# conanhujinming/flash_hash_join

Hardware: AMD Instinct MI355X
Metric: probe throughput (billion probes/sec), int64 keys, whole join (build + probe phases) per step (higher is better)
Workload: dtype int64

## Files before the change

flash_hash_join_amd/_lib.py:

```python
from __future__ import annotations

import ctypes
import os
import subprocess

_PKG = os.path.dirname(os.path.abspath(__file__))
VARIANT = os.environ.get("FJ_LIB_VARIANT", "")
LIB_PATH = (os.path.join(_PKG, "lib", "libflashjoin_hip.so") if not VARIANT
            else os.path.join(_PKG, "lib", "libflashjoin_hip_lab.so") if VARIANT == "lab"
            else os.path.join(_PKG, "lib", "ab", VARIANT + ".so"))
PRODUCT_LIB_PATH = os.path.join(_PKG, "lib", "libflashjoin_hip.so")
LAB_LIB_PATH = os.path.join(_PKG, "lib", "libflashjoin_hip_lab.so")
ABI_VERSION = 8
CSRC = os.path.join(_PKG, "csrc")

SYMBOLS = [
    "fj_initialize", "fj_last_error", "fj_device_count", "fj_version", "fj_abi_version", "fj_set_option", "fj_get_option", "fj_key_mix64", "fj_key_unmix64",
    "fj_ctx_create", "fj_ctx_destroy", "fj_ctx_workspace_bytes", "fj_ctx_trim",
    "fj_join_host", "fj_free_host", "fj_last_timings", "fj_join_device", "fj_emit_pairs",
    "fj_owner_split", "fj_stream_abort", "fj_shuffle_plan", "fj_bcast_plan",
    "fj_dist_comm_set_form", "fj_dist_model", "fj_dist_unique_id", "fj_dist_comm_create", "fj_dist_comm_from_nccl", "fj_dist_comm_from_transport",
    "fj_dist_comm_destroy", "fj_dist_comm_rank", "fj_dist_comm_size", "fj_dist_join_count", "fj_dist_join",
    "fj_generate_build", "fj_generate_probe",
    "fj_device_malloc", "fj_device_free", "fj_memcpy_h2d", "fj_memcpy_d2h", "fj_memcpy_d2d",
]
LAB_SYMBOLS = [
    "fj_owner_hist", "fj_owner_scatter",
    "fj_shuffle_chunk_bytes", "fj_shuffle_pack_begin", "fj_shuffle_pack_counts", "fj_shuffle_pack_finish", "fj_stream_open_shuffled",
    "fj_stream_append_build_chunks", "fj_stream_append_probe_chunks",
    "fj_shuffle_part_filter_bytes", "fj_shuffle_part_filter_range", "fj_stream_export_part_filters", "fj_shuffle_pack_filter", "fj_shuffle_pack_kept", "fj_part_filter_sample",
    "fj_bcast_region_bytes", "fj_bcast_piece_span", "fj_bcast_pack", "fj_bcast_pack_bounds", "fj_bcast_probe", "fj_bcast_join", "fj_bcast_finish", "fj_bcast_abort",
    "fj_bloom_filter_words", "fj_bloom_export", "fj_bloom_prefilter",
    "fj_stream_open", "fj_stream_append_build", "fj_stream_advance_probe", "fj_stream_begin", "fj_stream_append_probe", "fj_stream_finish",
    "fj_ctx_reserve_cus", "fj_key_pair64", "fj_debug_partition",
]


class FjTimings(ctypes.Structure):
    _fields_ = [
        ("total_ms", ctypes.c_double), ("build_phase_ms", ctypes.c_double), ("probe_phase_ms", ctypes.c_double),
        ("join_ms", ctypes.c_double), ("emit_ms", ctypes.c_double), ("probe_part_kernel_ms", ctypes.c_double * 4),
        ("h2d_ms", ctypes.c_double), ("d2h_ms", ctypes.c_double),
        ("path", ctypes.c_int), ("passes", ctypes.c_int), ("radix_bits", ctypes.c_int), ("fell_back", ctypes.c_int),
        ("partitions", ctypes.c_uint64), ("overlapped", ctypes.c_int), ("lds_retries", ctypes.c_int),
        ("filter_ms", ctypes.c_double), ("filter_survivors", ctypes.c_uint64), ("bloom_level", ctypes.c_int), ("sampled_hit_bp", ctypes.c_int), ("host_streamed", ctypes.c_int), ("reserved3", ctypes.c_int),
    ]

    def as_dict(self):
        d = {n: getattr(self, n) for n, _ in self._fields_ if n != "probe_part_kernel_ms"}
        d["probe_part_kernel_ms"] = list(self.probe_part_kernel_ms)
        return d


class FjDistTimings(ctypes.Structure):
    _fields_ = [
        ("struct_size", ctypes.c_size_t),
        ("total_ms", ctypes.c_double), ("split_ms", ctypes.c_double), ("exchange_ms", ctypes.c_double), ("join_ms", ctypes.c_double),
# ... 149 lines not shown
        L.fj_shuffle_chunk_bytes.restype = sz; L.fj_shuffle_chunk_bytes.argtypes = [sz, i32]
        L.fj_shuffle_pack_begin.restype = i32; L.fj_shuffle_pack_begin.argtypes = [vp, vp, vp, sz, sz, i32, i32, vp]
        L.fj_shuffle_part_filter_bytes.restype = sz; L.fj_shuffle_part_filter_bytes.argtypes = []
        L.fj_shuffle_part_filter_range.restype = i32; L.fj_shuffle_part_filter_range.argtypes = [sz, i32, i32, ctypes.POINTER(sz), ctypes.POINTER(sz), ctypes.POINTER(sz)]
        L.fj_stream_export_part_filters.restype = i32; L.fj_stream_export_part_filters.argtypes = [vp, vp, vp]
        L.fj_shuffle_pack_filter.restype = i32; L.fj_shuffle_pack_filter.argtypes = [vp, vp, vp]
        L.fj_shuffle_pack_kept.restype = u64; L.fj_shuffle_pack_kept.argtypes = [vp]
        L.fj_part_filter_sample.restype = i32; L.fj_part_filter_sample.argtypes = [vp, vp, sz, sz, vp, sz, i32, vp, pu64]
        L.fj_shuffle_pack_counts.restype = i32; L.fj_shuffle_pack_counts.argtypes = [vp, pu64]
        L.fj_shuffle_pack_finish.restype = i32; L.fj_shuffle_pack_finish.argtypes = [vp, ctypes.POINTER(vp), ctypes.POINTER(vp), ctypes.POINTER(vp), vp]
        L.fj_stream_open_shuffled.restype = i32; L.fj_stream_open_shuffled.argtypes = [vp, sz, i32, i32, sz, i32, sz, i32, i32, vp]
        L.fj_stream_append_build_chunks.restype = i32; L.fj_stream_append_build_chunks.argtypes = [vp, vp, vp, vp, sz, vp]
        L.fj_stream_append_probe_chunks.restype = i32; L.fj_stream_append_probe_chunks.argtypes = [vp, vp, vp, sz, vp]
        L.fj_bcast_region_bytes.restype = sz; L.fj_bcast_region_bytes.argtypes = [sz, sz, i32]
        L.fj_bcast_piece_span.restype = i32; L.fj_bcast_piece_span.argtypes = [sz, sz, sz, sz, i32, psz, psz]
        L.fj_bcast_pack.restype = i32; L.fj_bcast_pack.argtypes = [vp, vp, vp, sz, sz, vp, i32, i32, vp]
        L.fj_bcast_pack_bounds.restype = i32; L.fj_bcast_pack_bounds.argtypes = [vp, pu64]
        L.fj_bcast_probe.restype = i32; L.fj_bcast_probe.argtypes = [vp, vp, sz, sz, vp]
        L.fj_bcast_join.restype = i32; L.fj_bcast_join.argtypes = [vp, vp, i32, pu64, pu64, ctypes.c_uint32, ctypes.c_uint32, vp]
        L.fj_bcast_finish.restype = i32; L.fj_bcast_finish.argtypes = [vp, vp, pu64, ctypes.POINTER(FjTimings)]
        L.fj_bcast_abort.restype = None; L.fj_bcast_abort.argtypes = [vp]
        if hasattr(L, "fj_key_pair64"):
            L.fj_key_pair64.restype = u64; L.fj_key_pair64.argtypes = [u64, u64]
        L.fj_debug_partition.restype = i32
        L.fj_debug_partition.argtypes = [vp, vp, vp, sz, i32, i32, vp, vp, vp, vp, pu64]
    _lib = L
    return L


def last_error() -> str:
    return load().fj_last_error().decode("utf-8", "replace")


def check(rc: int) -> None:
    if rc != 0:
        msg = last_error()
        if "out of" in msg and "memory" in msg:
            raise MemoryError(msg)
        raise RuntimeError(msg)
```

flash_hash_join_amd/csrc/fj_host.h:

```cpp
#pragma once
#include "fj_internal.h"
#include "../../include/flashjoin.h"
#include "../../include/flashjoin_lab.h"

#include <algorithm>
#include <chrono>
#include <cstdarg>
#include <cstdio>
#include <cstdlib>
#include <cstring>
#include <condition_variable>
#include <functional>
#include <mutex>
#include <string>
#include <thread>
#include <vector>

struct StreamState;

namespace fjh {

int set_err(const char* fmt, ...);
fj_timings& last_timings();
#define HIPCHK(x)                                                                                          \
// ... 86 lines not shown

struct Prepared {
    enum Form { EMPTY, LDS, HBM };
    bool valid = false;
    Form form = EMPTY;
    bool has_vals = false;
    int top_bits = 64, path = 0;
    Plan plan; u32 nparts = 0;
    size_t nb = 0; u64 g = 0;
    u64* keys = nullptr; u64* rows = nullptr; u64* vals = nullptr; void* aux = nullptr;
    u64 cap_mask = 0;
    size_t bytes = 0;
};

struct PassIter {
    int side = 0; bool has_vals = false; size_t n = 0; Plan plan; int used = 64; u32 parents = 1; u64 lbound = 0;
    u32 tile_chunks = 16; int i = 0;
    FjChunkSet prev{}; bool have_prev = false; const uint4* tiles = nullptr; const u32* ntiles = nullptr; const u32* toff = nullptr;
    FjChunkSet cs{}; u32 Gmax = 1, F = 1, appends = 1;
    size_t piece_rows = 0;
    int slot = 0, cs_base = 0;
    u32 item_tc_max = 0;
    bool want_items = false; u32 items_cap = 0; u32* part_count = nullptr; int part_count_slot = W_PART_COUNT;
    bool bloom_done = false; const FjChunkSet* bloom_build = nullptr;
    const u32* bloom_prebuilt = nullptr;
    unsigned long long* bloom_bucket_keys = nullptr;
    int save_level = 0; FjChunkSet saved{};
    u32* alloc_word = nullptr; u32* seg_word = nullptr; u32* err_word = nullptr;
    bool in_pk7 = false; u32 in_b0 = 0, in_top_shift = 0;
    bool vals_pos = false;
};

}

struct PackState {
    bool begun = false, deferred = false;
    u32 part_shift = 0;
    fjh::PassIter it;
    FjPackArgs args{};
    int nranks = 0;
};

struct StreamState {
    bool active = false;
    fjh::Plan plan; fjh::PassIter pit, bit; FjLdsJoinArgs ja{};
    int top_bits = 64, evc = 0;
// ... 18 lines not shown
};

struct fj_ctx {
    int device = 0;
    fjh::Buf bufs[fjh::W_NSLOTS];
    hipEvent_t ev[fjh::E_NEV];
    hipStream_t side = nullptr;
    fjh::Scalars* d_sc = nullptr;
    fjh::Scalars* h_sc = nullptr;
    fjh::Pending pend;
    fjh::Prepared prep;
    StreamState st;
    PackState pk;
    BcastState bc;
    hipEvent_t pk_ev = nullptr;
    unsigned long long* pk_h = nullptr;
    size_t ws_bytes = 0;
    u32 num_cus = 256;
    u32 reserve_cus = 0;
    void* stage[3] = {nullptr, nullptr, nullptr};
    size_t stage_bytes = 0;
    bool plan_in_flight = false;
    bool slot_dirty[fjh::W_NSLOTS] = {};
    std::recursive_mutex mu;
};

namespace fjh {

#define FJ_HOOK_LOOPBACK 1
#define FJ_HOOK_INJECT_FAIL 2
#define FJ_HOOK_SPLIT_ALWAYS 4
#define FJ_HOOK_ONE_COMM 8
#define FJ_HOOK_RESERVE_ALWAYS 16
#define FJ_HOOK_EMIT_TAGGED 32
#define FJ_HOOK_EMIT_RETRY_7TH 64
struct Options {
    size_t radix_threshold = 0; int scalar_hbm_table = 0; u32 persistent_min_items = 8192; u32 plan_target_keys = FJ_PART_TARGET_KEYS;
    int bloom_variant = 0, bloom_auto = 1, bloom_auto_max_hit_bp = 2300, mat_single_pass = 1;
    int join_wide = 2;
    u32 lab_hooks = 0;
    u32 join_items_target = 2048;
    int mm_heavy_keys = 0;
    int mm_heavy_outer = 0;
    Options();
};
Options& options();

int get_buf(fj_ctx* c, int slot, size_t bytes, void** out);
int get_zeroed_buf(fj_ctx* c, int slot, size_t bytes, void** out, hipStream_t s);
int plan_npass(int bits);
void plan_passes(Plan& p, bool extra_first);
Plan make_plan(size_t nb, int top_bits, bool want_bloom = false, u64 target_override = 0);
void pass_init(PassIter& it, int side, bool has_vals, size_t n, const Plan& plan, int top_bits);
u32 pass_groups(u64 chunks, u64 rows, u32 tile_chunks, u32 F);
int pass_prepare(fj_ctx* c, PassIter& it, u32 appends, hipStream_t s);
int pass_launch(fj_ctx* c, PassIter& it, const u64* keys, const u64* vals, size_t n, hipStream_t s, int* ev_cursor);
bool bloom_stage_follows(const PassIter& it, int level);
void join_item_geometry(u64 nparts, size_t np, u64 chunk_bound, u32* tc, u64* max_items);
bool wide_join_planned(bool materialize, size_t nb, size_t np_eff, int bits);
int level_finish(fj_ctx* c, PassIter& it, bool final_level, hipStream_t s);
int pass_complete(fj_ctx* c, PassIter& it, hipStream_t s);
int bloom_stage(fj_ctx* c, PassIter& it, hipStream_t s);
int run_passes(fj_ctx* c, PassIter& it, const u64* keys, const u64* vals, hipStream_t s, FjChunkSet* out, int* ev_cursor);
int clear_plan_scalars(fj_ctx* c, hipStream_t s);
void begin_plan(fj_ctx* c);
void end_plan(fj_ctx* c);
void drop_pending(fj_ctx* c);
int begin_step(fj_ctx* c, const char* who);
int read_scalars(fj_ctx* c, hipStream_t s);
float ev_ms(fj_ctx* c, int a, int b);
void plan_timings(fj_ctx* c, const Plan& plan, u64 partitions, int evc, fj_timings* t);
int stamps_begin(unsigned long long** dbg, hipStream_t s);
int stamps_report(const char* label, const unsigned long long* dbg, u32 nitems, hipStream_t s);

int emit_pending(fj_ctx* c, u64* d_ok, u64* d_ov, size_t cap, hipStream_t s, fj_timings* t);
int radix_join_tail(fj_ctx* c, int materialize, FjLdsJoinArgs& ja, const Plan& plan, size_t np, const PassIter& pit, hipStream_t s,
                    fj_timings* t, int evc, u64* out_count, bool* lds_full, int top_bits, SingleOut* so = nullptr);

int join_outer(fj_ctx* c, int mode, bool use_radix, const u64* bk, const u64* bv, size_t nb, const u64* pk, size_t np, int top_bits,
               hipStream_t s, fj_timings* t, u64* out_count, u64* d_ok, u64* d_ov, bool rid = false);
int join_full(fj_ctx* c, bool use_radix, const u64* bk, const u64* bv, size_t nb, const u64* pk, size_t np, int top_bits,
// ... 42 lines not shown
```

flash_hash_join_amd/csrc/fj_internal.h:

```cpp
#pragma once
#include "fj_common.h"

#define FJ_ERR_POOL 1u
#define FJ_ERR_LDS_FULL 2u
#define FJ_STAT_DUPS 4u
#define FJ_STAT_RETRY 8u
#define FJ_STAT_EMIT_RETRY 16u
#define FJ_ERR_VARIANT 32u
#define FJ_BLOOM_HDR_MAGIC 0xB100F000u
#define FJ_STAT_TOOBIG 64u
#define FJ_ERR_OUTCAP 128u
#define FJ_ERR_PAIR_COLLISION 256u
#define FJ_ITEM_RETRY 0xFFFFFFFFu
#define FJ_ITEM_TOOBIG 0xFFFFFFFEu

struct FjPartArgs {
    const u64* in_keys;
    const u64* in_vals;
    const u32* in_list;
    const u32* in_dir;
    const uint4* in_tiles;
    const u32* in_ntiles;
    u64 n_flat;
    u32 parent0;
// ... 18 lines not shown
};

struct FjChunkSet {
    u64* keys;
    u64* vals;
    u64 n_flat;
    u32* dir;
    u64* rel;
    u32* seg_off;
    u32* alloc;
    u32 cap;
    u32 nb;
    u32 fan_mask;
    u32 max_segs;
    u32* bchunks;
    u32* boff;
    u32* list;
    u32 run_log;
};

u32 fj_partition_lds_bytes(u32 fan_log, bool vals, int line_log);
u32 fj_partition_tile_chunks(u32 fan_log, bool vals);
hipError_t fj_launch_partition(const FjPartArgs& a, bool vals, int line_log, u32 grid, hipStream_t s);
hipError_t fj_launch_group(const FjChunkSet& cs, u32 tc, u32* toff, uint4* tiles, u32 max_tiles, u32* zero_tail, hipStream_t s);
hipError_t fj_launch_scan_u32_to_u64(const u32* in, u64* out, u32 n, hipStream_t s);
hipError_t fj_launch_dir_rank(u32* dir, u32 n, u32 b_lo, u32 nbk, u32 fan, u64* rel, u32* seg_off, u32* bchunks, u32* nalloc, hipStream_t s);

struct FjBloomArgs {
    const u64* pkeys;
    const u32* plist;
    const uint4* tiles;
    u64* out_keys; u32* out_dir; u64* out_rel;
    u32 cap_chunks;
    u32 pnb;
    const u32* toff;
    const u64* bkeys; const u32* blist; const u32* bboff;
    u32* seg_off; u32* bchunks; u32* alloc; u32* seg_counter;
    u32 max_segs;
    u32* err;
    unsigned long long* survivors;
    const u32* prebuilt;
    unsigned long long* bucket_keys;
};
u32 fj_bloom_tile_chunks();
u32 fj_bloom_waves_per_group();
u32 fj_bloom_slab_chunks();
hipError_t fj_launch_bloom_filter(const FjBloomArgs& a, u32 grid, int variant, hipStream_t s);
// ... 229 lines not shown
```

flash_hash_join_amd/csrc/fj_joins.hip:

```cpp
#include "fj_host.h"

namespace fjh {

static int skew_side(fj_ctx* c, PassIter& it, int side, bool vals, const FjChunkSet& in, const std::vector<u32>& off, u64 chunks, int S, int bits_left,
                     int slot, int tiles_slot, u32* d_nt, hipStream_t s);

int emit_pending(fj_ctx* c, u64* d_ok, u64* d_ov, size_t cap, hipStream_t s, fj_timings* t) {
    Pending& pd = c->pend;
    if (!pd.valid) return set_err("fj_emit_pairs: no counted materialising join is pending on this context");
    if (pd.count > cap) return set_err("fj_emit_pairs: output capacity %zu < %llu pairs", cap, (unsigned long long)pd.count);
    if (pd.count > 0 && (((uintptr_t)d_ok | (uintptr_t)d_ov) & 7)) return set_err("output buffers must be 8-byte aligned");
    HIPCHK(hipEventRecord(c->ev[E_EMIT0], s));
    if (pd.count > 0) {
        void* p;
        if (pd.kind == Pending::LDS) {
            if (pd.lds.row_ids) {
                pd.lds.dedup = 1; pd.lds.orig_vals = nullptr;
            } else if (pd.has_dups) {
                if (get_buf(c, W_ROWIDX, pd.nb * 8, &p)) return 1;
                u64* rowidx = (u64*)p;
                HIPCHK(fj_launch_iota(rowidx, pd.nb, s));
                HIPCHK(hipMemsetAsync(&c->d_sc->alloc[0], 0, sizeof(c->d_sc->alloc) + sizeof(c->d_sc->seg_counter), s));
                PassIter bit;
                pass_init(bit, 0, true, pd.nb, make_plan(pd.nb, pd.top_bits), pd.top_bits);
// ... 321 lines not shown
            HIPCHK(hipMemcpy(h.data(), jw.dbg, h.size() * 8, hipMemcpyDeviceToHost));
            double acc[8] = {0, 0, 0, 0, 0, 0, 0, 0};
            for (u32 g = 0; g < grid && g < 4096; ++g) for (int i = 0; i < 8; ++i) acc[i] += (double)h[g * 8 + i] * 0.01;
            u32 nit = 0;
            HIPCHK(hipMemcpy(&nit, jw.nitems_dev, 4, hipMemcpyDeviceToHost));
            const double per = (double)std::min<u32>(grid, 4096) * ((double)nit / grid);
            fprintf(stderr, "[FJ_WIDE_STAMPS] us per item (thread 0): rotate+requests %.3f  claim_issue+zero %.3f  barB %.3f  probe %.3f  resolve+park %.3f  barA %.3f  stores %.3f\n",
                    acc[0] / per, acc[5] / per, acc[6] / per, acc[1] / per, acc[2] / per, acc[3] / per, acc[4] / per);
            for (int ph = 0; ph < 3; ++ph) {
                fprintf(stderr, "[FJ_WIDE_STAMPS] wave 0..15, %s:", ph == 0 ? "requests + claims issued + probe" : ph == 1 ? "claims resolved + park (to barrier A)" : "stores (barrier A to B)");
                for (int w = 0; w < 16; ++w) {
                    double sacc = 0;
                    for (u32 g = 0; g < grid && g < 256; ++g) sacc += (double)h[2048 * 8 + g * 64 + w * 4 + ph] * 0.01;
                    fprintf(stderr, " %.2f", sacc / ((double)std::min<u32>(grid, 256) * ((double)nit / grid)));
                }
                fprintf(stderr, "\n");
            }
        }
    } else
    HIPCHK(fj_launch_lds_join(ja, false, s, &c->d_sc->next_item, options().persistent_min_items));
    if (ja.dbg) { if (stamps_report("FJ_JOIN_STAMPS", ja.dbg, nitems, s)) return 1; ja.dbg = nullptr; }
    HIPCHK(hipEventRecord(c->ev[E_JOIN], s));
    if (read_scalars(c, s)) return 1;
    t->lds_retries = 0;
    if ((c->h_sc->err & FJ_STAT_RETRY) && !(c->h_sc->err & (FJ_ERR_POOL | FJ_ERR_LDS_FULL))) {
        ja.retry_only = 1; ja.mark_toobig = ja.items ? 1u : 0u;
        HIPCHK(fj_launch_lds_join_retry(ja, s));
        ja.retry_only = 0;
        HIPCHK(hipEventRecord(c->ev[E_JOIN], s));
        if (read_scalars(c, s)) return 1;
        t->lds_retries = 1;
        if ((c->h_sc->err & FJ_STAT_TOOBIG) && !(c->h_sc->err & (FJ_ERR_POOL | FJ_ERR_LDS_FULL))) {
            bool ok = false; u32 redone = 0;
            if (skew_join(c, ja, plan, top_bits, nitems, pit.slot, materialize, s, &ok, &redone, &c->pend)) return 1;
            HIPCHK(hipEventRecord(c->ev[E_JOIN], s));
            if (read_scalars(c, s)) return 1;
            if (ok) t->lds_retries = 1 + (int)redone;
            else c->h_sc->err |= FJ_ERR_LDS_FULL;
        }
    }
    if (c->h_sc->err & FJ_ERR_POOL) return set_err("internal error: chunk pool exhausted during a partition pass");
    end_plan(c);
    plan_timings(c, plan, ja.nparts, evc, t);
    if (c->h_sc->err & FJ_ERR_LDS_FULL) { *lds_full = true; return 0; }
    *out_count = c->h_sc->total;
    if (materialize) {
// ... 15 lines not shown
    HIPCHK(hipEventRecord(c->ev[E_START], s));
    if (clear_plan_scalars(c, s)) return 1;
    FjLdsJoinArgs ja{};
    PassIter bit, pit;
    pass_init(bit, 0, materialize != 0, nb, plan, top_bits);
    bit.vals_pos = rid;
    int evc = 0;
    if (plan.bloom_level > 0) bit.save_level = plan.bloom_level;
    if (run_passes(c, bit, bk, (materialize && !rid) ? bv : nullptr, s, &ja.build, nullptr)) return 1;
    HIPCHK(hipEventRecord(c->ev[E_BUILD], s));
    Plan pplan = plan;
    if (bloom == 2) {
        const u32 nsamp = FJ_SAMPLE_KEYS;
        HIPCHK(fj_launch_sample_hits(ja.build, pk, np, nsamp, (u32)(top_bits - 32 - plan.bits), (1u << plan.bits) - 1u, &c->d_sc->sample_hits, s));
        HIPCHK(hipMemcpyAsync(&c->h_sc->sample_hits, &c->d_sc->sample_hits, sizeof(unsigned long long), hipMemcpyDeviceToHost, s));
        HIPCHK(hipStreamSynchronize(s));
        const u32 hit_bp = (u32)(c->h_sc->sample_hits * 10000ull / nsamp);
        t->sampled_hit_bp = (int)hit_bp;
        if (hit_bp > (u32)options().bloom_auto_max_hit_bp) { pplan = make_plan(nb, top_bits, false); plan.bloom_level = 0; plan.npass = pplan.npass; }
    }
    pass_init(pit, 1, rid, np, pplan, top_bits);
    pit.vals_pos = rid;
    pit.want_items = true;
    {
        size_t np_eff = np;
        if (plan.bloom_level > 0) np_eff = (size_t)((double)np * (t->sampled_hit_bp >= 0 ? std::min(10000, t->sampled_hit_bp + 1000) : 1500) / 10000.0);
        if (wide_join_planned(materialize != 0, nb, np_eff, plan.bits)) pit.item_tc_max = 32;
    }
    if (plan.bloom_level > 0) pit.bloom_build = &bit.saved;
    if (run_passes(c, pit, pk, nullptr, s, &ja.probe, &evc)) return 1;
    HIPCHK(hipEventRecord(c->ev[E_PPART], s));
    ja.avg_build_keys = (u32)std::min<u64>(0xFFFFFFFFu, (u64)nb >> plan.bits);
    ja.row_ids = rid ? 1u : 0u;
    if (radix_join_tail(c, materialize, ja, plan, np, pit, s, t, evc, out_count, lds_full, top_bits, so)) return 1;
    if (c->pend.valid) { c->pend.bk = bk; c->pend.bv = bv; c->pend.nb = nb; c->pend.top_bits = top_bits; }
    return 0;
}

static int mm_tile_join(fj_ctx* c, const FjLdsJoinArgs& ja, u32 nitems, int materialize, hipStream_t s, Pending* pend,
                        int outer = FJ_MM_INNER, const FjMmOuterArgs* oa = nullptr) {
    u32 nlive = 0;
    std::vector<u32> pc(nitems), boff((size_t)ja.build.nb + 1);
    std::vector<uint4> items(nitems);
    HIPCHK(hipMemcpyAsync(&nlive, ja.nitems_dev, 4, hipMemcpyDeviceToHost, s));
    HIPCHK(hipMemcpyAsync(pc.data(), ja.part_count, (size_t)nitems * 4, hipMemcpyDeviceToHost, s));
    HIPCHK(hipMemcpyAsync(items.data(), ja.items, (size_t)nitems * sizeof(uint4), hipMemcpyDeviceToHost, s));
// ... 628 lines not shown
```

flash_hash_join_amd/csrc/fj_partition.hip:

```cpp
#include "fj_internal.h"
#include <cstdlib>
#include <mutex>
#include <vector>

namespace {

#ifndef FJ_LO_PAD
#define FJ_LO_PAD 1u
#endif
struct PartLds {
    u32 sorted_k, sorted_v, lo_k, lo_v, hist, toff, line_desc, t_chunk, t_cnt, wsum, misc, total;
};
__host__ __device__ inline PartLds part_lds_layout(u32 T, u32 F, u32 line, bool vals, u32 nwaves) {
    PartLds L;
    const u32 nsorted = T + 2;
    const u32 maxl = (T + (line - 1) * F) / line + 2;
    u32 o = 0;
    L.sorted_k = o; o += nsorted * 8;
    L.sorted_v = o; if (vals) o += nsorted * 8;
    L.lo_k = o; o += F * (line + FJ_LO_PAD) * 8;
    L.lo_v = o; if (vals) o += F * (line + FJ_LO_PAD) * 8;
    L.line_desc = o; o += maxl * 8;
    L.wsum = o; o += nwaves * 8;
    L.hist = o; o += (F + 4) * 4;
// ... 438 lines not shown
            inc[j] = v;
            if (lane == 63) wtot[j][wave] = v;
        }
        __syncthreads();
        T before = carry, total = carry;
#pragma unroll
        for (int j = 0; j < 4; ++j) {
            T mine = 0, all = 0;
            for (u32 w = 0; w < 16; ++w) { const T c = wtot[j][w]; all += c; if (w < wave) mine += c; }
            T run = total + mine + inc[j] - sum[j];
            const u32 e0 = base + 4u * ((u32)j * 1024u + tid);
#pragma unroll
            for (int k = 0; k < 4; ++k) { if (e0 + k < n) put(e0 + k, run); run += x[j][k]; }
            total += all;
        }
        (void)before;
        carry = total;
        __syncthreads();
    }
    return carry;
}

__global__ __launch_bounds__(1024) void fj_level_scan(u32* __restrict__ bchunks, u32* __restrict__ boff, u32 n, u32 tc,
                                                      u32* __restrict__ toff) {
    __shared__ u64 wtot[4][16];
    const u32 tid = threadIdx.x, lane = tid & 63, wave = tid >> 6;
    const float rtc = tc ? 1.0f / (float)tc : 0.f;
    auto tiles_of = [&](u32 c) -> u32 {
        if (!tc) return 0u;
        u32 q = (u32)((float)c * rtc);
        while (q * tc < c) ++q;
        while (q && (q - 1) * tc >= c) --q;
        return q;
    };
    u64 carry = 0;
    for (u32 base = 0; base < n; base += 16384) {
        uint4 x[4]; u64 sum[4], inc[4];
#pragma unroll
        for (int j = 0; j < 4; ++j) {
            const u32 e0 = base + 4u * ((u32)j * 1024u + tid);
            x[j] = make_uint4(0, 0, 0, 0);
            if (e0 < n) { x[j] = *reinterpret_cast<const uint4*>(bchunks + e0); *reinterpret_cast<uint4*>(bchunks + e0) = make_uint4(0, 0, 0, 0); }
            sum[j] = ((u64)x[j].x + x[j].y + x[j].z + x[j].w) | ((u64)(tiles_of(x[j].x) + tiles_of(x[j].y) + tiles_of(x[j].z) + tiles_of(x[j].w)) << 32);
            u64 v = sum[j];
#pragma unroll
            for (int d = 1; d < 64; d <<= 1) { const u64 y = __shfl_up(v, d, 64); if ((int)lane >= d) v += y; }
            inc[j] = v;
            if (lane == 63) wtot[j][wave] = v;
        }
        __syncthreads();
        u64 total = carry;
#pragma unroll
        for (int j = 0; j < 4; ++j) {
            u64 mine = 0, all = 0;
            for (u32 w = 0; w < 16; ++w) { const u64 c = wtot[j][w]; all += c; if (w < wave) mine += c; }
            u64 run = total + mine + inc[j] - sum[j];
// ... 146 lines not shown
                const u32 i = i0 + u * stride;
                e[u] = i < n ? dir[i] : FJ_DIR_INVALID;
                r[u] = i < n ? rel[i] : 0;
            }
            u32 pos[4]; bool ok[4];
#pragma unroll
            for (int u = 0; u < 4; ++u) {
                const u32 b = e[u] >> FJ_DIR_CNT_BITS, seg = (u32)(r[u] >> 32);
                ok[u] = e[u] != FJ_DIR_INVALID && seg < max_segs;
                pos[u] = ok[u] ? boff[b] + seg_off[(u64)seg * (fan_mask + 1) + (b & fan_mask)] + (u32)r[u] : 0;
            }
#pragma unroll
            for (int u = 0; u < 4; ++u)
                if (ok[u]) list[pos[u]] = (((e[u] & FJ_DIR_CNT_MASK) - 1u) << 24) | (i0 + u * stride);
        }
    }
}

template <bool FUSED>
__global__ __launch_bounds__(1024) void fj_level_lists_binned(const u32* __restrict__ dir, const u64* __restrict__ rel, const u32* __restrict__ nalloc,
                               u32 cap, u32* __restrict__ boff_g, const u32* __restrict__ seg_off, u32 fan_mask,
                               u32 max_segs, u32* __restrict__ list,
                               u32 nb, u32 tc, u32* __restrict__ toff_g, uint4* __restrict__ tiles, u32 max_tiles,
                               u32* __restrict__ zero_tail, u32* __restrict__ bchunks) {
    constexpr u32 NT = 1024, BLK = 4096, NBMAX = 512;
    __shared__ u32 hist[NBMAX + 1];
    __shared__ u32 wsum[NBMAX / 64];
    __shared__ uint2 ent[BLK];
    __shared__ u32 boff_s[FUSED ? NBMAX + 1 : 1], toff_s[FUSED ? NBMAX + 1 : 1];
    __shared__ u64 wtot[NBMAX / 64];
    __shared__ u32 s_last;
    const u32* boff = FUSED ? boff_s : boff_g;
    const u32* toff = FUSED ? toff_s : toff_g;
    u32 n = *nalloc; if (n > cap) n = cap;
    const u32 tid = threadIdx.x, lane = tid & 63, wave = tid >> 6;
    const u32 stride = gridDim.x * NT, gtid = blockIdx.x * NT + tid;
    if constexpr (FUSED) {
        const float rtc = tc ? 1.0f / (float)tc : 0.f;
        auto tiles_of = [&](u32 c) -> u32 {
            if (!tc) return 0u;
            u32 q = (u32)((float)c * rtc);
            while (q * tc < c) ++q;
            while (q && (q - 1) * tc >= c) --q;
            return q;
        };
        u64 mine = 0, v = 0;
        if (tid < NBMAX) {
            const u32 c = tid < nb ? bchunks[tid] : 0u;
            mine = (u64)c | ((u64)tiles_of(c) << 32);
            v = mine;
#pragma unroll
            for (int d = 1; d < 64; d <<= 1) { const u64 y = __shfl_up(v, d, 64); if ((int)lane >= d) v += y; }
            if (lane == 63) wtot[wave] = v;
        }
        __syncthreads();
        if (tid == 0) { __threadfence(); s_last = atomicAdd(&bchunks[nb], 1u) == gridDim.x - 1 ? 1u : 0u; }
        if (tid < NBMAX) {
            u64 woff = 0;
            for (u32 w = 0; w < wave; ++w) woff += wtot[w];
            const u64 ex = woff + v - mine;
            if (tid < nb) { boff_s[tid] = (u32)ex; toff_s[tid] = (u32)(ex >> 32); }
            if (tid == nb - 1) { boff_s[nb] = (u32)(ex + mine); toff_s[nb] = (u32)((ex + mine) >> 32); }
        }
        __syncthreads();
        if (s_last) { if (tid < nb) bchunks[tid] = 0; if (tid == 0) bchunks[nb] = 0; }
        if (blockIdx.x == 0 && tid <= nb) { boff_g[tid] = boff_s[tid]; if (tc) toff_g[tid] = toff_s[tid]; }
    }
// ... 166 lines not shown
    if (a.fan_log > FJ_MAX_FAN_LOG || a.slab < (1u << FJ_RUN_LOG) || (a.slab & ((1u << FJ_RUN_LOG) - 1u))) return hipErrorInvalidValue;
    if (a.in_pk7) {
        if (!a.in_list || a.run_log != FJ_RUN_LOG) return hipErrorInvalidValue;
        if (vals) {
            if (a.fan_log == 9 && line_log != 3) return hipErrorInvalidValue;
            return line_log == 3 ? launch_part0<1024, 4, 3, true, false, true, FJ_RUN_LOG, true>(a, grid, s)
                                 : launch_part0<1024, 4, 4, true, false, true, FJ_RUN_LOG, true>(a, grid, s);
        }
        if (line_log != 4) return hipErrorInvalidValue;
        const u32 g = a.fan_log == 9 ? grid : (grid < 256 ? grid : 256);
        return a.side == 0 ? launch_part0<1024, 8, 4, false, false, false, FJ_RUN_LOG, true>(a, g, s)
                           : launch_part0<1024, 8, 4, false, false, true, FJ_RUN_LOG, true>(a, g, s);
    }
    if (a.fan_log == 9) {
        if (vals) return line_log == 3 ? launch_part2<1024, 4, true>(a, 3, grid, s) : hipErrorInvalidValue;
        return launch_part2<1024, 8, false>(a, line_log, grid, s);
    }
    if (vals) {
        return launch_part2<1024, 4, true>(a, line_log, grid, s);
    }
    return launch_part2<1024, 8, false>(a, line_log, grid < 256 ? grid : 256, s);
}

hipError_t fj_launch_group(const FjChunkSet& cs, u32 tc, u32* toff, uint4* tiles, u32 max_tiles, u32* zero_tail, hipStream_t s) {
    if (cs.nb & 3u) return hipErrorInvalidValue;
    static_assert(FJ_RUN_LOG == 1 || FJ_RUN_LOG == 2, "fj_level_lists reads a run's directory words with one 8-B or 16-B load");
    if (cs.run_log != 0 && cs.run_log != FJ_RUN_LOG) return hipErrorInvalidValue;
    if (cs.run_log == 0 && cs.nb <= 512 && cs.cap >= 4096) {
        const u32 blocks = (cs.cap + 4095u) / 4096u;
        if (blocks <= 512u) {
            hipLaunchKernelGGL(fj_level_lists_binned<true>, dim3(blocks), dim3(1024), 0, s, cs.dir, cs.rel, cs.alloc, cs.cap, cs.boff,
                               cs.seg_off, cs.fan_mask, cs.max_segs, cs.list, cs.nb, tc, toff, tiles, max_tiles, zero_tail, cs.bchunks);
        } else {
            hipLaunchKernelGGL(fj_level_scan, dim3(1), dim3(1024), 0, s, cs.bchunks, cs.boff, cs.nb, tc, toff);
            hipLaunchKernelGGL(fj_level_lists_binned<false>, dim3(blocks < 4096u ? blocks : 4096u), dim3(1024), 0, s, cs.dir, cs.rel, cs.alloc, cs.cap, cs.boff,
                               cs.seg_off, cs.fan_mask, cs.max_segs, cs.list, cs.nb, tc, toff, tiles, max_tiles, zero_tail, cs.bchunks);
        }
        return hipGetLastError();
    }
    const bool wide = cs.nb >= 8192u && cs.nb <= (1u << 19);
    if (wide) hipLaunchKernelGGL(fj_level_scan_wide, dim3((cs.nb + 4095u) / 4096u), dim3(1024), 0, s, cs.bchunks, cs.boff, cs.nb, tc, toff);
    else hipLaunchKernelGGL(fj_level_scan, dim3(1), dim3(1024), 0, s, cs.bchunks, cs.boff, cs.nb, tc, toff);
    auto kern = cs.run_log ? fj_level_lists<FJ_RUN_LOG> : fj_level_lists<0>;
    hipLaunchKernelGGL(kern, dim3(2048), dim3(256), 0, s, cs.dir, cs.rel, cs.alloc, cs.cap, cs.boff, cs.seg_off,
                       cs.fan_mask, cs.max_segs, cs.list, cs.nb, tc, toff, tiles, max_tiles, zero_tail, wide ? cs.bchunks : (u32*)nullptr);
    return hipGetLastError();
}

hipError_t fj_launch_dir_rank(u32* dir, u32 n, u32 b_lo, u32 nbk, u32 fan, u64* rel, u32* seg_off, u32* bchunks, u32* nalloc, hipStream_t s) {
    if (nbk > (1u << FJ_MAX_FAN_LOG) || fan < nbk || n == 0) return hipErrorInvalidValue;
    hipLaunchKernelGGL(fj_dir_rank_kernel, dim3((n + 4095u) / 4096u), dim3(1024), 0, s, dir, n, b_lo, nbk, fan, rel, seg_off, bchunks, nalloc);
    return hipGetLastError();
}

hipError_t fj_launch_scan_u32_to_u64(const u32* in, u64* out, u32 n, hipStream_t s) {
    hipLaunchKernelGGL(fj_scan_u32_to_u64, dim3(1), dim3(1024), 0, s, in, out, n);
    return hipGetLastError();
}
```

flash_hash_join_amd/csrc/fj_plan.hip:

```cpp
#include "fj_host.h"

namespace fjh {

namespace { thread_local std::string g_err; thread_local fj_timings g_last; }

int set_err(const char* fmt, ...) {
    char buf[1024];
    va_list ap; va_start(ap, fmt); vsnprintf(buf, sizeof buf, fmt, ap); va_end(ap);
    g_err = buf;
    return 1;
}
fj_timings& last_timings() { return g_last; }

Options& options() { static Options o; return o; }
static int set_option_value(Options& o, const char* name, long long value);
Options::Options() {
    static const char* const legacy[] = {"FJ_RADIX_THRESHOLD", "FJ_SCALAR_HBM_TABLE", "FJ_BLOOM_AUTO", "FJ_BLOOM_AUTO_MAX_HIT_BP", "FJ_BLOOM_VARIANT", "FJ_PLAN_TARGET_KEYS",
                                         "FJ_MAT_SINGLE_PASS", "FJ_PERSISTENT_MIN_ITEMS", "FJ_JOIN_ITEMS_TARGET", "FJ_JOIN_WIDE", "FJ_DIST_LOOPBACK", "FJ_DIST_INJECT_FAIL",
                                         "FJ_DIST_RESERVE_ALWAYS", "FJ_DIST_SPLIT_ALWAYS", "FJ_DIST_ONE_COMM", "FJ_EMIT_TAGGED"};
    for (const char* name : legacy)
        if (getenv(name)) fprintf(stderr, "flash_hash_join_amd: the environment variable %s is no longer read (use FJ_OPTIONS=\"name=value,...\" or fj_set_option; see include/flashjoin.h)\n", name);
    const char* e = getenv("FJ_OPTIONS");
    if (!e) return;
    std::string str(e);
// ... 129 lines not shown
        a.in_keys = it.prev.keys; a.in_vals = it.prev.vals; a.in_list = it.prev.list; a.in_dir = it.prev.dir;
        a.in_tiles = it.tiles; a.in_ntiles = it.ntiles; a.n_flat = 0;
    } else {
        a.in_keys = keys; a.in_vals = vals; a.in_list = nullptr; a.in_dir = nullptr; a.in_tiles = nullptr; a.in_ntiles = nullptr; a.n_flat = n;
        a.vals_pos = it.has_vals && it.vals_pos ? 1u : 0u;
        G = std::min(G, pass_groups((n + FJ_CHUNK - 1) / FJ_CHUNK, n, it.tile_chunks, it.F));
    }
    a.parent0 = 0;
    a.out_keys = cs.keys; a.out_vals = cs.vals; a.out_dir = cs.dir; a.out_rel = cs.rel; a.seg_off = cs.seg_off;
    a.bchunks = cs.bchunks; a.alloc = cs.alloc; a.seg_counter = it.seg_word ? it.seg_word : &c->d_sc->seg_counter[it.side * 4 + it.i];
    a.cap_chunks = cs.cap; a.max_segs = cs.max_segs;
    a.err = it.err_word ? it.err_word : &c->d_sc->err;
    if (it.have_prev && it.in_pk7) { a.in_pk7 = 1; a.in_b0 = it.in_b0; a.in_top_shift = it.in_top_shift; }
    a.shift = (u32)it.used; a.fan_log = (u32)it.plan.fan_log[it.i]; a.slab = fj_slab_for(it.appends); a.run_log = cs.run_log; a.side = (u32)it.side;
    const int line_log = (it.has_vals && it.F > 256) ? 3 : 4;
    if (ev_cursor) HIPCHK(hipEventRecord(c->ev[E_PK0 + 2 * (*ev_cursor)], s));
    HIPCHK(fj_launch_partition(a, it.has_vals, line_log, G, s));
    if (ev_cursor) { HIPCHK(hipEventRecord(c->ev[E_PK0 + 2 * (*ev_cursor) + 1], s)); ++*ev_cursor; }
    return 0;
}

bool bloom_stage_follows(const PassIter& it, int level) { return it.plan.bloom_level == level && it.bloom_build && !it.bloom_done; }

void join_item_geometry(u64 nparts, size_t np, u64 chunk_bound, u32* tc, u64* max_items) {
    const u64 pchunks = (np + FJ_CHUNK - 1) / FJ_CHUNK;
    const u64 bound = std::max<u64>(chunk_bound, pchunks);
    const u64 avg = std::max<u64>(1, bound / nparts);
    u64 want = 1;
    const u64 target_items = options().join_items_target;
    if (nparts < target_items) want = std::min<u64>((target_items + nparts - 1) / nparts, std::max<u64>(1, (pchunks / nparts) / 32));
    *tc = (u32)(want > 1 ? std::max<u64>(8, (avg * 9 / 8 + want - 1) / want) : std::max<u64>(512, 4 * avg));
    *max_items = bound / *tc + nparts + 1;
}

bool wide_join_planned(bool materialize, size_t nb, size_t np_eff, int bits) {
    if (materialize || bits <= 0 || options().join_wide == 0) return false;
    if (options().join_wide == 1) return true;
    return np_eff <= 3 * nb;
}

int level_finish(fj_ctx* c, PassIter& it, bool final_level, hipStream_t s) {
    const FjChunkSet& cs = it.cs;
    u32 tc = 0; u64 max_tiles = 0; u32* zero_tail = nullptr;
    if (bloom_stage_follows(it, it.i)) tc = fj_bloom_tile_chunks();
    else if (!final_level) tc = fj_partition_tile_chunks((u32)it.plan.fan_log[it.i], it.has_vals);
    else if (it.want_items) {
        join_item_geometry(cs.nb, it.n, it.lbound, &tc, &max_tiles);
        if (it.item_tc_max && tc > it.item_tc_max) { tc = it.item_tc_max; max_tiles = std::max<u64>(it.lbound, (it.n + FJ_CHUNK - 1) / FJ_CHUNK) / tc + cs.nb + 1; }
    }
    if (tc && !max_tiles) max_tiles = it.lbound / tc + cs.nb + 1;
    if (max_tiles >= (1ull << 31)) return set_err("internal error: tile table too large");
    u32* toff = nullptr; uint4* tiles = nullptr;
    void* p;
    if (tc) {
        if (get_buf(c, it.cs_base + W_TOFF, ((size_t)cs.nb + 1) * 4, &p)) return 1; toff = (u32*)p;
        if (get_buf(c, it.cs_base + W_TILES, max_tiles * sizeof(uint4), &p)) return 1; tiles = (uint4*)p;
        if (final_level) {
            if (get_buf(c, it.part_count_slot, (size_t)max_tiles * 4, &p)) return 1;
            it.part_count = zero_tail = (u32*)p; it.items_cap = (u32)max_tiles;
        }
    }
    HIPCHK(fj_launch_group(cs, tc, toff, tiles, (u32)max_tiles, zero_tail, s));
    it.tiles = tiles; it.ntiles = toff ? toff + cs.nb : nullptr; it.toff = toff;
    return 0;
}

int pass_complete(fj_ctx* c, PassIter& it, hipStream_t s) {
    const FjChunkSet& cs = it.cs;
    it.lbound = it.n / FJ_CHUNK + 1 + (u64)(it.Gmax + it.parents) * it.F * it.appends;
    ++it.i;
    if (level_finish(c, it, it.i == it.plan.npass, s)) return 1;
    it.prev = cs; it.have_prev = true;
    it.parents = cs.nb;
    ++it.slot;
    if (it.save_level == it.i) it.saved = cs;
    return 0;
}

int bloom_stage(fj_ctx* c, PassIter& it, hipStream_t s) {
    const FjChunkSet in = it.prev;
    const u32 G = c->num_cus;
    const u32 nw = fj_bloom_waves_per_group();
    const u64 max_segs = (u64)nw * ((u64)in.nb + G) + 16;
    const u64 cap64 = it.n / FJ_CHUNK + 1 + max_segs + (u64)fj_bloom_slab_chunks() * nw * G;
    if (cap64 >= (1ull << 24)) return set_err("relation of %zu rows is too large for one GPU's chunk directory", it.n);
// ... 269 lines not shown
    u64 w = 0;
    for (u32 b = 0; b < cs.nb; ++b) {
        for (u32 i = boff[b]; i < boff[b + 1]; ++i) {
            const u32 id = FJ_LIST_ID(list[i]);
            if (id >= cs.cap) return set_err("fj_debug_partition: list entry %u out of range", id);
            const u32 e = dir[id], cnt = e & FJ_DIR_CNT_MASK;
            if ((e >> FJ_DIR_CNT_BITS) != b) return set_err("fj_debug_partition: chunk %u listed under bucket %u but tagged %u", id, b, e >> FJ_DIR_CNT_BITS);
            if (cnt == 0 || cnt > FJ_CHUNK || cnt != FJ_LIST_CNT(list[i])) return set_err("fj_debug_partition: chunk %u has count %u (list says %u)", id, cnt, FJ_LIST_CNT(list[i]));
            if (w + cnt > n) return set_err("fj_debug_partition: more than %zu rows in the chunk lists", n);
            HIPCHK(hipMemcpy(ck.data(), cs.keys + (size_t)id * FJ_CHUNK, cnt * 8, hipMemcpyDeviceToHost));
            for (u32 j = 0; j < cnt; ++j) h_out_keys[w + j] = fj_key_unmix(ck[j]);
            if (d_vals && h_out_vals) {
                HIPCHK(hipMemcpy(cv.data(), cs.vals + (size_t)id * FJ_CHUNK, cnt * 8, hipMemcpyDeviceToHost));
                memcpy(h_out_vals + w, cv.data(), cnt * 8);
            }
            for (u32 j = 0; j < cnt; ++j) h_bucket_of[w + j] = b;
            w += cnt;
        }
    }
    *h_nvalid = w;
    return 0;
}

int fj_device_malloc(void** p, size_t bytes) { HIPCHK(hipMalloc(p, bytes ? bytes : 16)); return 0; }
int fj_device_free(void* p) { if (p) HIPCHK(hipFree(p)); return 0; }
int fj_memcpy_h2d(void* d, const void* h, size_t bytes) { if (bytes) HIPCHK(hipMemcpy(d, h, bytes, hipMemcpyHostToDevice)); return 0; }
int fj_memcpy_d2h(void* h, const void* d, size_t bytes) { if (bytes) HIPCHK(hipMemcpy(h, d, bytes, hipMemcpyDeviceToHost)); return 0; }
int fj_memcpy_d2d(void* dst, const void* src, size_t bytes) { if (bytes) HIPCHK(hipMemcpy(dst, src, bytes, hipMemcpyDeviceToDevice)); return 0; }

void fj_free_host(void* p) { free(p); }
int fj_last_timings(fj_timings* out) { if (!out) return set_err("fj_last_timings: null"); *out = last_timings(); return 0; }

}
```

include/flashjoin_lab.h:

```cpp
#ifndef FLASHJOIN_LAB_H
#define FLASHJOIN_LAB_H
#include "flashjoin.h"

#ifdef __cplusplus
extern "C" {
#endif
#if defined(__GNUC__)
#pragma GCC visibility push(default)
#endif

int fj_owner_hist(fj_ctx* ctx, const uint64_t* d_keys, size_t n, int nranks, uint64_t* h_counts, void* stream);
int fj_owner_scatter(fj_ctx* ctx, const uint64_t* d_keys, const uint64_t* d_vals, size_t n, int nranks, const uint64_t* h_counts,
                     uint64_t* d_out_keys, uint64_t* d_out_vals, void* stream);

size_t fj_shuffle_chunk_bytes(size_t nb_total, int nranks);
int fj_shuffle_pack_begin(fj_ctx* ctx, const uint64_t* d_keys, const uint64_t* d_vals, size_t n, size_t nb_total, int nranks, int defer_plan, void* stream);
int fj_shuffle_pack_counts(fj_ctx* ctx, uint64_t* h_used);
int fj_shuffle_pack_finish(fj_ctx* ctx, void* const* d_dst_chunks, uint64_t* const* d_dst_vals, uint32_t* const* d_dst_dir, void* stream);
int fj_stream_open_shuffled(fj_ctx* ctx, size_t nb_total, int nranks, int rank, size_t nb_bound, int build_appends,
                            size_t np_bound, int probe_appends, int with_vals, void* stream);
int fj_stream_append_build_chunks(fj_ctx* ctx, const void* d_chunks, const uint64_t* d_vals, uint32_t* d_dir, size_t nchunks, void* stream);
int fj_stream_append_probe_chunks(fj_ctx* ctx, const void* d_chunks, uint32_t* d_dir, size_t nchunks, void* stream);
size_t fj_shuffle_part_filter_bytes(void);
int fj_shuffle_part_filter_range(size_t nb_total, int nranks, int rank, size_t* first_part, size_t* n_parts, size_t* total_parts);
// ... 14 lines not shown

size_t fj_bloom_filter_words(void);
int fj_bloom_export(fj_ctx* ctx, const uint64_t* d_build_keys, size_t nb, int hash_top_bits, uint32_t* d_filters, void* stream);
int fj_bloom_prefilter(fj_ctx* ctx, const uint64_t* d_probe_keys, size_t n, int hash_top_bits, const uint32_t* d_filters,
                       uint64_t* d_out_keys, size_t out_capacity, uint64_t* out_n, void* stream);

int fj_stream_open(fj_ctx* ctx, size_t nb_bound, int build_appends, size_t np_bound, int probe_appends, void* stream,
                   int hash_top_bits);
int fj_stream_append_build(fj_ctx* ctx, const uint64_t* d_build_keys, size_t n, void* stream);
int fj_stream_advance_probe(fj_ctx* ctx, void* stream);
int fj_stream_begin(fj_ctx* ctx, const uint64_t* d_build_keys, const uint64_t* d_build_vals, size_t nb, size_t np_bound,
                    int max_appends, void* stream, int hash_top_bits);
int fj_stream_append_probe(fj_ctx* ctx, const uint64_t* d_probe_keys, size_t n, void* stream);
int fj_stream_finish(fj_ctx* ctx, void* stream, uint64_t* out_count, fj_timings* timings);

void fj_ctx_reserve_cus(fj_ctx* ctx, unsigned n);

uint64_t fj_key_pair64(uint64_t a, uint64_t b);

int fj_debug_partition(fj_ctx* ctx, const uint64_t* d_keys, const uint64_t* d_vals, size_t n, int total_bits,
                       int hash_top_bits, void* stream, uint64_t* h_out_keys, uint64_t* h_out_vals,
                       uint32_t* h_bucket_of, uint64_t* h_nvalid);


#if defined(__GNUC__)
#pragma GCC visibility pop
#endif
#ifdef __cplusplus
}
#endif
#endif
```

Baseline: 116.1.

## Size join work items to resident wave count and enforce minimum slices per partition

```diff
diff --git a/flash_hash_join_amd/_lib.py b/flash_hash_join_amd/_lib.py
--- a/flash_hash_join_amd/_lib.py
+++ b/flash_hash_join_amd/_lib.py
@@ -32,7 +32,7 @@
     "fj_bcast_region_bytes", "fj_bcast_piece_span", "fj_bcast_pack", "fj_bcast_pack_bounds", "fj_bcast_probe", "fj_bcast_join", "fj_bcast_finish", "fj_bcast_abort",
     "fj_bloom_filter_words", "fj_bloom_export", "fj_bloom_prefilter",
     "fj_stream_open", "fj_stream_append_build", "fj_stream_advance_probe", "fj_stream_begin", "fj_stream_append_probe", "fj_stream_finish",
-    "fj_ctx_reserve_cus", "fj_key_pair64", "fj_debug_partition",
+    "fj_ctx_reserve_cus", "fj_key_pair64", "fj_debug_partition", "fj_debug_item_counts",
 ]
 
 
@@ -228,6 +228,8 @@
         L.fj_bcast_abort.restype = None; L.fj_bcast_abort.argtypes = [vp]
         if hasattr(L, "fj_key_pair64"):
             L.fj_key_pair64.restype = u64; L.fj_key_pair64.argtypes = [u64, u64]
+        if hasattr(L, "fj_debug_item_counts"):
+            L.fj_debug_item_counts.restype = i32; L.fj_debug_item_counts.argtypes = [vp, vp, vp, vp, sz, pu64]
         L.fj_debug_partition.restype = i32
         L.fj_debug_partition.argtypes = [vp, vp, vp, sz, i32, i32, vp, vp, vp, vp, pu64]
     _lib = L
diff --git a/flash_hash_join_amd/csrc/fj_host.h b/flash_hash_join_amd/csrc/fj_host.h
--- a/flash_hash_join_amd/csrc/fj_host.h
+++ b/flash_hash_join_amd/csrc/fj_host.h
@@ -132,6 +132,7 @@
     int slot = 0, cs_base = 0;
     u32 item_tc_max = 0;
     bool want_items = false; u32 items_cap = 0; u32* part_count = nullptr; int part_count_slot = W_PART_COUNT;
+    bool items_per_resident = false;
     bool bloom_done = false; const FjChunkSet* bloom_build = nullptr;
     const u32* bloom_prebuilt = nullptr;
     unsigned long long* bloom_bucket_keys = nullptr;
@@ -196,6 +197,7 @@
     size_t stage_bytes = 0;
     bool plan_in_flight = false;
     bool slot_dirty[fjh::W_NSLOTS] = {};
+    std::vector<u32> dbg_item_counts, dbg_item_parts, dbg_item_chunks;
     std::recursive_mutex mu;
 };
 
@@ -208,6 +210,8 @@
 #define FJ_HOOK_RESERVE_ALWAYS 16
 #define FJ_HOOK_EMIT_TAGGED 32
 #define FJ_HOOK_EMIT_RETRY_7TH 64
+#define FJ_HOOK_ITEMS_BY_TARGET 128
+#define FJ_HOOK_SNAPSHOT_ITEMS 256
 struct Options {
     size_t radix_threshold = 0; int scalar_hbm_table = 0; u32 persistent_min_items = 8192; u32 plan_target_keys = FJ_PART_TARGET_KEYS;
     int bloom_variant = 0, bloom_auto = 1, bloom_auto_max_hit_bp = 2300, mat_single_pass = 1;
@@ -230,7 +234,7 @@
 int pass_prepare(fj_ctx* c, PassIter& it, u32 appends, hipStream_t s);
 int pass_launch(fj_ctx* c, PassIter& it, const u64* keys, const u64* vals, size_t n, hipStream_t s, int* ev_cursor);
 bool bloom_stage_follows(const PassIter& it, int level);
-void join_item_geometry(u64 nparts, size_t np, u64 chunk_bound, u32* tc, u64* max_items);
+void join_item_geometry(u64 nparts, size_t np, u64 chunk_bound, u32* tc, u64* max_items, u32 resident, u32* min_slices);
 bool wide_join_planned(bool materialize, size_t nb, size_t np_eff, int bits);
 int level_finish(fj_ctx* c, PassIter& it, bool final_level, hipStream_t s);
 int pass_complete(fj_ctx* c, PassIter& it, hipStream_t s);
diff --git a/flash_hash_join_amd/csrc/fj_internal.h b/flash_hash_join_amd/csrc/fj_internal.h
--- a/flash_hash_join_amd/csrc/fj_internal.h
+++ b/flash_hash_join_amd/csrc/fj_internal.h
@@ -64,7 +64,7 @@
 u32 fj_partition_lds_bytes(u32 fan_log, bool vals, int line_log);
 u32 fj_partition_tile_chunks(u32 fan_log, bool vals);
 hipError_t fj_launch_partition(const FjPartArgs& a, bool vals, int line_log, u32 grid, hipStream_t s);
-hipError_t fj_launch_group(const FjChunkSet& cs, u32 tc, u32* toff, uint4* tiles, u32 max_tiles, u32* zero_tail, hipStream_t s);
+hipError_t fj_launch_group(const FjChunkSet& cs, u32 tc, u32* toff, uint4* tiles, u32 max_tiles, u32* zero_tail, hipStream_t s, u32 want = 0);
 hipError_t fj_launch_scan_u32_to_u64(const u32* in, u64* out, u32 n, hipStream_t s);
 hipError_t fj_launch_dir_rank(u32* dir, u32 n, u32 b_lo, u32 nbk, u32 fan, u64* rel, u32* seg_off, u32* bchunks, u32* nalloc, hipStream_t s);
 
diff --git a/flash_hash_join_amd/csrc/fj_joins.hip b/flash_hash_join_amd/csrc/fj_joins.hip
--- a/flash_hash_join_amd/csrc/fj_joins.hip
+++ b/flash_hash_join_amd/csrc/fj_joins.hip
@@ -367,6 +367,18 @@
     if (ja.dbg) { if (stamps_report("FJ_JOIN_STAMPS", ja.dbg, nitems, s)) return 1; ja.dbg = nullptr; }
     HIPCHK(hipEventRecord(c->ev[E_JOIN], s));
     if (read_scalars(c, s)) return 1;
+    if ((options().lab_hooks & FJ_HOOK_SNAPSHOT_ITEMS) && ja.items && !materialize) {
+        u32 nlive = 0;
+        HIPCHK(hipMemcpy(&nlive, ja.nitems_dev, 4, hipMemcpyDeviceToHost));
+        if (nlive > nitems) nlive = nitems;
+        std::vector<uint4> items(nlive);
+        c->dbg_item_counts.assign(nlive, 0); c->dbg_item_parts.assign(nlive, 0); c->dbg_item_chunks.assign(nlive, 0);
+        if (nlive) {
+            HIPCHK(hipMemcpy(c->dbg_item_counts.data(), ja.part_count, (size_t)nlive * 4, hipMemcpyDeviceToHost));
+            HIPCHK(hipMemcpy(items.data(), ja.items, (size_t)nlive * sizeof(uint4), hipMemcpyDeviceToHost));
+        }
+        for (u32 i = 0; i < nlive; ++i) { c->dbg_item_parts[i] = items[i].z; c->dbg_item_chunks[i] = items[i].y; }
+    }
     t->lds_retries = 0;
     if ((c->h_sc->err & FJ_STAT_RETRY) && !(c->h_sc->err & (FJ_ERR_POOL | FJ_ERR_LDS_FULL))) {
         ja.retry_only = 1; ja.mark_toobig = ja.items ? 1u : 0u;
@@ -428,6 +440,7 @@
     pass_init(pit, 1, rid, np, pplan, top_bits);
     pit.vals_pos = rid;
     pit.want_items = true;
+    pit.items_per_resident = !materialize && !(options().lab_hooks & FJ_HOOK_ITEMS_BY_TARGET);
     {
         size_t np_eff = np;
         if (plan.bloom_level > 0) np_eff = (size_t)((double)np * (t->sampled_hit_bp >= 0 ? std::min(10000, t->sampled_hit_bp + 1000) : 1500) / 10000.0);
diff --git a/flash_hash_join_amd/csrc/fj_partition.hip b/flash_hash_join_amd/csrc/fj_partition.hip
--- a/flash_hash_join_amd/csrc/fj_partition.hip
+++ b/flash_hash_join_amd/csrc/fj_partition.hip
@@ -484,7 +484,7 @@
 }
 
 __global__ __launch_bounds__(1024) void fj_level_scan(u32* __restrict__ bchunks, u32* __restrict__ boff, u32 n, u32 tc,
-                                                      u32* __restrict__ toff) {
+                                                      u32* __restrict__ toff, u32 want) {
     __shared__ u64 wtot[4][16];
     const u32 tid = threadIdx.x, lane = tid & 63, wave = tid >> 6;
     const float rtc = tc ? 1.0f / (float)tc : 0.f;
@@ -493,7 +493,8 @@
         u32 q = (u32)((float)c * rtc);
         while (q * tc < c) ++q;
         while (q && (q - 1) * tc >= c) --q;
-        return q;
+        const u32 w = (c + 31u) >> 5 < want ? (c + 31u) >> 5 : want;
+        return q > w ? q : w;
     };
     u64 carry = 0;
     for (u32 base = 0; base < n; base += 16384) {
@@ -686,7 +687,7 @@
                                u32 cap, u32* __restrict__ boff_g, const u32* __restrict__ seg_off, u32 fan_mask,
                                u32 max_segs, u32* __restrict__ list,
                                u32 nb, u32 tc, u32* __restrict__ toff_g, uint4* __restrict__ tiles, u32 max_tiles,
-                               u32* __restrict__ zero_tail, u32* __restrict__ bchunks) {
+                               u32* __restrict__ zero_tail, u32* __restrict__ bchunks, u32 want) {
     constexpr u32 NT = 1024, BLK = 4096, NBMAX = 512;
     __shared__ u32 hist[NBMAX + 1];
     __shared__ u32 wsum[NBMAX / 64];
@@ -706,7 +707,8 @@
             u32 q = (u32)((float)c * rtc);
             while (q * tc < c) ++q;
             while (q && (q - 1) * tc >= c) --q;
-            return q;
+            const u32 w = (c + 31u) >> 5 < want ? (c + 31u) >> 5 : want;
+            return q > w ? q : w;
         };
         u64 mine = 0, v = 0;
         if (tid < NBMAX) {
@@ -919,25 +921,26 @@
     return launch_part2<1024, 8, false>(a, line_log, grid < 256 ? grid : 256, s);
 }
 
-hipError_t fj_launch_group(const FjChunkSet& cs, u32 tc, u32* toff, uint4* tiles, u32 max_tiles, u32* zero_tail, hipStream_t s) {
+hipError_t fj_launch_group(const FjChunkSet& cs, u32 tc, u32* toff, uint4* tiles, u32 max_tiles, u32* zero_tail, hipStream_t s, u32 want) {
     if (cs.nb & 3u) return hipErrorInvalidValue;
+    if (want && (!tc || want > tc || want > 16u || cs.nb >= 8192u)) return hipErrorInvalidValue;
     static_assert(FJ_RUN_LOG == 1 || FJ_RUN_LOG == 2, "fj_level_lists reads a run's directory words with one 8-B or 16-B load");
     if (cs.run_log != 0 && cs.run_log != FJ_RUN_LOG) return hipErrorInvalidValue;
     if (cs.run_log == 0 && cs.nb <= 512 && cs.cap >= 4096) {
         const u32 blocks = (cs.cap + 4095u) / 4096u;
         if (blocks <= 512u) {
             hipLaunchKernelGGL(fj_level_lists_binned<true>, dim3(blocks), dim3(1024), 0, s, cs.dir, cs.rel, cs.alloc, cs.cap, cs.boff,
-                               cs.seg_off, cs.fan_mask, cs.max_segs, cs.list, cs.nb, tc, toff, tiles, max_tiles, zero_tail, cs.bchunks);
+                               cs.seg_off, cs.fan_mask, cs.max_segs, cs.list, cs.nb, tc, toff, tiles, max_tiles, zero_tail, cs.bchunks, want);
         } else {
-            hipLaunchKernelGGL(fj_level_scan, dim3(1), dim3(1024), 0, s, cs.bchunks, cs.boff, cs.nb, tc, toff);
+            hipLaunchKernelGGL(fj_level_scan, dim3(1), dim3(1024), 0, s, cs.bchunks, cs.boff, cs.nb, tc, toff, want);
             hipLaunchKernelGGL(fj_level_lists_binned<false>, dim3(blocks < 4096u ? blocks : 4096u), dim3(1024), 0, s, cs.dir, cs.rel, cs.alloc, cs.cap, cs.boff,
-                               cs.seg_off, cs.fan_mask, cs.max_segs, cs.list, cs.nb, tc, toff, tiles, max_tiles, zero_tail, cs.bchunks);
+                               cs.seg_off, cs.fan_mask, cs.max_segs, cs.list, cs.nb, tc, toff, tiles, max_tiles, zero_tail, cs.bchunks, want);
         }
         return hipGetLastError();
     }
     const bool wide = cs.nb >= 8192u && cs.nb <= (1u << 19);
     if (wide) hipLaunchKernelGGL(fj_level_scan_wide, dim3((cs.nb + 4095u) / 4096u), dim3(1024), 0, s, cs.bchunks, cs.boff, cs.nb, tc, toff);
-    else hipLaunchKernelGGL(fj_level_scan, dim3(1), dim3(1024), 0, s, cs.bchunks, cs.boff, cs.nb, tc, toff);
+    else hipLaunchKernelGGL(fj_level_scan, dim3(1), dim3(1024), 0, s, cs.bchunks, cs.boff, cs.nb, tc, toff, want);
     auto kern = cs.run_log ? fj_level_lists<FJ_RUN_LOG> : fj_level_lists<0>;
     hipLaunchKernelGGL(kern, dim3(2048), dim3(256), 0, s, cs.dir, cs.rel, cs.alloc, cs.cap, cs.boff, cs.seg_off,
                        cs.fan_mask, cs.max_segs, cs.list, cs.nb, tc, toff, tiles, max_tiles, zero_tail, wide ? cs.bchunks : (u32*)nullptr);
diff --git a/flash_hash_join_amd/csrc/fj_plan.hip b/flash_hash_join_amd/csrc/fj_plan.hip
--- a/flash_hash_join_amd/csrc/fj_plan.hip
+++ b/flash_hash_join_amd/csrc/fj_plan.hip
@@ -175,15 +175,17 @@
 
 bool bloom_stage_follows(const PassIter& it, int level) { return it.plan.bloom_level == level && it.bloom_build && !it.bloom_done; }
 
-void join_item_geometry(u64 nparts, size_t np, u64 chunk_bound, u32* tc, u64* max_items) {
+void join_item_geometry(u64 nparts, size_t np, u64 chunk_bound, u32* tc, u64* max_items, u32 resident, u32* min_slices) {
     const u64 pchunks = (np + FJ_CHUNK - 1) / FJ_CHUNK;
     const u64 bound = std::max<u64>(chunk_bound, pchunks);
     const u64 avg = std::max<u64>(1, bound / nparts);
     u64 want = 1;
-    const u64 target_items = options().join_items_target;
+    if (resident && nparts < resident && (pchunks / nparts) / 32 < (resident + nparts - 1) / nparts) resident = 0;
+    const u64 target_items = resident ? resident : options().join_items_target;
     if (nparts < target_items) want = std::min<u64>((target_items + nparts - 1) / nparts, std::max<u64>(1, (pchunks / nparts) / 32));
     *tc = (u32)(want > 1 ? std::max<u64>(8, (avg * 9 / 8 + want - 1) / want) : std::max<u64>(512, 4 * avg));
-    *max_items = bound / *tc + nparts + 1;
+    *min_slices = (resident && want > 1 && want <= 16 && want <= *tc && nparts < 8192) ? (u32)want : 0u;
+    *max_items = bound / *tc + nparts * std::max<u64>(1, *min_slices) + 1;
 }
 
 bool wide_join_planned(bool materialize, size_t nb, size_t np_eff, int bits) {
@@ -194,12 +196,12 @@
 
 int level_finish(fj_ctx* c, PassIter& it, bool final_level, hipStream_t s) {
     const FjChunkSet& cs = it.cs;
-    u32 tc = 0; u64 max_tiles = 0; u32* zero_tail = nullptr;
+    u32 tc = 0; u64 max_tiles = 0; u32* zero_tail = nullptr; u32 min_slices = 0;
     if (bloom_stage_follows(it, it.i)) tc = fj_bloom_tile_chunks();
     else if (!final_level) tc = fj_partition_tile_chunks((u32)it.plan.fan_log[it.i], it.has_vals);
     else if (it.want_items) {
-        join_item_geometry(cs.nb, it.n, it.lbound, &tc, &max_tiles);
-        if (it.item_tc_max && tc > it.item_tc_max) { tc = it.item_tc_max; max_tiles = std::max<u64>(it.lbound, (it.n + FJ_CHUNK - 1) / FJ_CHUNK) / tc + cs.nb + 1; }
+        join_item_geometry(cs.nb, it.n, it.lbound, &tc, &max_tiles, it.items_per_resident ? 2 * c->num_cus : 0u, &min_slices);
+        if (it.item_tc_max && tc > it.item_tc_max) { tc = it.item_tc_max; min_slices = 0; max_tiles = std::max<u64>(it.lbound, (it.n + FJ_CHUNK - 1) / FJ_CHUNK) / tc + cs.nb + 1; }
     }
     if (tc && !max_tiles) max_tiles = it.lbound / tc + cs.nb + 1;
     if (max_tiles >= (1ull << 31)) return set_err("internal error: tile table too large");
@@ -213,7 +215,7 @@
             it.part_count = zero_tail = (u32*)p; it.items_cap = (u32)max_tiles;
         }
     }
-    HIPCHK(fj_launch_group(cs, tc, toff, tiles, (u32)max_tiles, zero_tail, s));
+    HIPCHK(fj_launch_group(cs, tc, toff, tiles, (u32)max_tiles, zero_tail, s, min_slices));
     it.tiles = tiles; it.ntiles = toff ? toff + cs.nb : nullptr; it.toff = toff;
     return 0;
 }
@@ -529,6 +531,18 @@
     return 0;
 }
 
+int fj_debug_item_counts(fj_ctx* c, uint32_t* h_counts, uint32_t* h_parts, uint32_t* h_chunks, size_t cap, uint64_t* h_n) {
+    if (!h_n) return set_err("fj_debug_item_counts: null");
+    FJ_ENTER(c);
+    const size_t n = c->dbg_item_counts.size();
+    *h_n = n;
+    if (n > cap) return set_err("fj_debug_item_counts: %zu items, room for %zu", n, cap);
+    if (n && h_counts) memcpy(h_counts, c->dbg_item_counts.data(), n * 4);
+    if (n && h_parts) memcpy(h_parts, c->dbg_item_parts.data(), n * 4);
+    if (n && h_chunks) memcpy(h_chunks, c->dbg_item_chunks.data(), n * 4);
+    return 0;
+}
+
 int fj_device_malloc(void** p, size_t bytes) { HIPCHK(hipMalloc(p, bytes ? bytes : 16)); return 0; }
 int fj_device_free(void* p) { if (p) HIPCHK(hipFree(p)); return 0; }
 int fj_memcpy_h2d(void* d, const void* h, size_t bytes) { if (bytes) HIPCHK(hipMemcpy(d, h, bytes, hipMemcpyHostToDevice)); return 0; }
diff --git a/include/flashjoin_lab.h b/include/flashjoin_lab.h
--- a/include/flashjoin_lab.h
+++ b/include/flashjoin_lab.h
@@ -60,6 +60,7 @@
                        int hash_top_bits, void* stream, uint64_t* h_out_keys, uint64_t* h_out_vals,
                        uint32_t* h_bucket_of, uint64_t* h_nvalid);
 
+int fj_debug_item_counts(fj_ctx* ctx, uint32_t* h_counts, uint32_t* h_parts, uint32_t* h_chunks, size_t cap, uint64_t* h_n);
 
 #if defined(__GNUC__)
 #pragma GCC visibility pop
```

Result: no change. 116.0 (-0.1%).
